# yahoo/bftkv

Measured on AMD Instinct MI355X. Metric: pgp_rsa2048_signature_verifies_per_sec, higher is better.
Workload: dtype u32; 1 GPU; 64-replica quorum, 10000 RSA-2048 signed writes per GPU (cfg2 of BASELINE.json), 534164 signature packets per GPU, 1.0% corrupt / 0.5% unknown issuer / 0.5% duplicate / 1.0% one-short; parallelism=shard-by-write x1, RCCL all-gather of verdict bitmaps on the verifier's stream, replicas=64, writes_per_gpu=10000, sigs_per_gpu=534164, batches_in_flight=3

## Files before the change

bftkv_amd/csrc/capi.hip:

```cpp
#include "../../include/bftkv_gpu.h"

#include <hip/hip_runtime.h>
#include <stdio.h>
#include <stdlib.h>
#include <string.h>

#include <limits.h>
#include <linux/futex.h>
#include <sched.h>
#include <sys/syscall.h>
#include <unistd.h>

#include <algorithm>
#include <array>
#include <atomic>
#include <memory>
#include <functional>
#include <map>
#include <set>
#include <chrono>
#include <condition_variable>
#include <mutex>
#include <shared_mutex>
#include <system_error>
// ... 163 lines not shown
  DevBuf txt_mid32, txt_mid64, txt_tail, txt_len;
  DevBuf forced_iss;
  DevBuf counts, base, total, item_flags, walk_scratch, cert_ent, sig_class, mid, mid64, hash_mask, recs, digests, r, xr, pk_list, pk_list3072, pk_list4096, r3072, r4096, pk_count, dsa_list, dsa_u, ids_tmp;
  DevBuf o_err, o_nver, o_verdict, o_fenced;
  DevBuf in_tbs, in_tbs_off, in_ss, in_ss_off;
  hipEvent_t seg_ev = nullptr;
  DevBuf in_prefix, in_prefix_off, in_shared, in_shared_off, in_seg;
  DevBuf st_tmp, item_tmp, bits_tmp, plan_cut;
  DevBuf chunk_arena, chunk_ctr;
  uint32_t multiexp_parts = 0;
  uint32_t ec_split = 0;
  uint32_t ec_window = 0;
  DevBuf ec_fb_tab[4];
  uint32_t ec_fb_w[4] = {};
  uint32_t multiexp_block = 0;
  uint32_t multiexp_lanes = 0;
  uint32_t rsav_lanes = 0;
  uint32_t dsa_inv_mode = 0;
  bool psign_caller_order = false;
  uint32_t n_cus = 256;
  uint32_t lagrange_x_bound = 0;
  bool early_exit = true;
  std::vector<DevBuf*> scratch_pool;
  std::unordered_map<std::string, std::vector<uint32_t>> modrow_cache;
  std::unordered_map<std::string, std::vector<uint32_t>> rsav_row_cache[2];
  std::map<std::string, std::array<DevBuf, 4>> modtab_cache;
  uint32_t* h_mail = nullptr;
  uint32_t* d_mail = nullptr;
  uint32_t last_total = 0, last_rsa = 0, last_items = 0;
  bool last_total_on_dev = false;
  hipEvent_t ev[10] = {};
  hipEvent_t ev_turn = nullptr;
  bool have_timing = false;
  void* rccl_comm = nullptr;
  int n_ranks = 1, rank = 0;

  bftkv_gpu_ctx* root = nullptr;
  std::shared_mutex kt_rw;
  std::atomic<int> kt_writers{0};
  std::atomic<int> n_forks{0};
  uint64_t quorum_gen = 0;
  uint64_t seen_keyring_gen = ~0ull, seen_quorum_gen = ~0ull;
  size_t n_dsa_slots = 0;
  int kt_read_depth = 0;
  DevBuf in_pack;
  uint8_t* h_out = nullptr; uint8_t* d_out = nullptr; size_t out_cap = 0;
  uint32_t out_seq = 0;
  std::vector<bftkv_gpu_ctx*> hb_workers;
  hipStream_t stream_c = nullptr;
  hipStream_t stream_c2 = nullptr;
  std::vector<hipEvent_t> hb_ev;
  uint8_t* hb_out = nullptr; size_t hb_out_cap = 0;
  uint32_t modexp_lds_pad = 0;
  uint32_t hb_pieces = 0;
  hipEvent_t hb_ev0 = nullptr;
  bool hb_tight = false;
  uint32_t hb_copy_mode = 0;
  void* hb_ring = nullptr;
  std::vector<float> hb_trace;
  uint32_t hb_last_pieces = 0;
  std::vector<uint32_t> hb_item0;
  void* small_pin = nullptr;
  uint32_t staged_spin_us = 50000;
};

void rccl_release(bftkv_gpu_ctx* c);
void release_small_pin(bftkv_gpu_ctx* c);
extern "C" int signature_verify_entities(bftkv_gpu_ctx* c, uint32_t n_items, const uint8_t* tbs, const uint64_t* tbs_off, const uint8_t* sig,
                                         const uint64_t* sig_off, const uint32_t* ent, uint8_t* err_out, const uint8_t* sig_class = nullptr,
                                         uint8_t* fenced_out = nullptr, const uint64_t* forced_issuer = nullptr);

namespace {

int fork_refresh(bftkv_gpu_ctx* c);

struct KtWrite {
  bftkv_gpu_ctx* c;
  explicit KtWrite(bftkv_gpu_ctx* c_) : c(c_) { c->kt_writers.fetch_add(1); c->kt_rw.lock(); }
  ~KtWrite() { c->kt_rw.unlock(); c->kt_writers.fetch_sub(1); }
};
struct KtRead {
  bftkv_gpu_ctx *c, *r;
  int rc = 0;
  explicit KtRead(bftkv_gpu_ctx* c_) : c(c_), r(c_->root) {
    if (!r || c->kt_read_depth++ > 0) return;
    while (r->kt_writers.load(std::memory_order_acquire) > 0) std::this_thread::yield();
    r->kt_rw.lock_shared();
    rc = fork_refresh(c);
  }
  ~KtRead() { if (r && --c->kt_read_depth == 0) r->kt_rw.unlock_shared(); }
};

struct Turnstile { std::mutex mu; hipEvent_t last = nullptr; const void* owner = nullptr; };
Turnstile g_turnstile[16];
constexpr uint64_t HB_PIPE_MIN_BYTES = 24ull << 20;
constexpr uint32_t HB_PIPE_MAX_PIECES = 8;
std::mutex g_hb_mu[16];
constexpr size_t HB_TR = 10;
struct HbRing {
  static constexpr size_t SLOT = 16u << 20;
  static constexpr int NSLOT = 6;
  static constexpr int THREADS = 4;
  uint8_t* base = nullptr;
  hipEvent_t ev[NSLOT] = {};
  bool used[NSLOT] = {};
  ~HbRing() { if (base) (void)hipHostFree(base); for (auto e : ev) if (e) (void)hipEventDestroy(e); }
// ... 276 lines not shown
  }
  uint32_t* const cnt_p = c->pk_count.as<uint32_t>();
  const uint32_t* const start0 = cnt_p + 12;
  PlanArgs pl{};
  if (total && plan_q) {
    pl.recs = c->recs.as<SigRec>(); pl.rec_base = c->base.as<uint32_t>(); pl.counts = c->counts.as<uint32_t>(); pl.n_items = n_items;
    pl.pk_list = c->pk_list.as<uint32_t>(); pl.dsa_list = c->dsa_list.as<uint32_t>(); pl.pk_list3072 = c->pk_list3072.as<uint32_t>();
    pl.pk_list4096 = c->pk_list4096.as<uint32_t>(); pl.pk_count = cnt_p; pl.plan_cut = c->plan_cut.as<uint32_t>(); pl.verdict = nullptr;
    int min_suff = 0;
    for (int i = 0; i < plan_q->n_qcs; ++i) if (plan_q->suff[i] > 0 && (min_suff == 0 || plan_q->suff[i] < min_suff)) min_suff = plan_q->suff[i];
    pl.margin = 1u + (uint32_t)min_suff / 64u;
    pl.mail = c->d_mail ? c->d_mail + 3 : nullptr;
    if (c->h_mail) __atomic_store_n(&c->h_mail[3], 0u, __ATOMIC_RELEASE);
    hipLaunchKernelGGL(k_plan<1>, dim3((n_items + PLAN_ITEMS - 1) / PLAN_ITEMS), dim3(PLAN_BLOCK), 0, s, pl, c->kt, *plan_q);
  }
  const bool dsa_side = total && c->have_dsa_keys;
  if (one_stream && dsa_side) HIPCHK(c, hipEventRecord(c->ev[1], s)); else HIPCHK(c, rec(1, s));
  const size_t n_slots = c->root ? c->n_dsa_slots : c->dsa_comb_slot.size();
  const uint32_t inv_batch_min = c->dsa_inv_mode == 1 || n_slots > (c->dsa_inv_mode == 2 ? (size_t)INV_MAX_SLOTS : 256) ? 0xFFFFFFFFu
                                 : c->dsa_inv_mode == 2 ? 0u : (uint32_t)std::max<size_t>(4096, 64 * n_slots);
  auto launch_dsa_inv = [&](hipStream_t st, const uint32_t* start) {
    if (inv_batch_min != 0xFFFFFFFFu)
      hipLaunchKernelGGL(k_dsa_inv_batched, dim3((total + INV_TILE - 1) / INV_TILE), dim3(INV_BLOCK), 0, st, d_ss, c->recs.as<SigRec>(),
                         c->dsa_list.as<uint32_t>(), c->pk_count.as<uint32_t>(), start, c->kt, c->dsa_u.as<uint32_t>(), inv_batch_min);
    if (inv_batch_min != 0u)
      hipLaunchKernelGGL(k_dsa_inv, dim3((total + 63) / 64), dim3(64), 0, st, d_ss, c->recs.as<SigRec>(), c->dsa_list.as<uint32_t>(),
                         c->pk_count.as<uint32_t>(), start, c->kt, c->dsa_u.as<uint32_t>(), inv_batch_min);
  };
  if (total && c->have_dsa_keys) {
    HIPCHK(c, hipStreamWaitEvent(c->stream_d, c->ev[1], 0));
    launch_dsa_inv(c->stream_d, start0);
    HIPCHK(c, hipEventRecord(c->ev[7], c->stream_d));
  }
  auto hash_stream_work = [&]() -> int {
    HIPCHK(c, join(sh, 1));
    if (total) {
      if (!d_mid_in) {
        hipLaunchKernelGGL(k_hash_mid_other, dim3((n_items + 63) / 64, N_HASHES - 1), dim3(64), 0, sh, d_tbs, d_tbs_off, n_items,
                           c->hash_mask.as<uint32_t>(), c->mid.as<uint32_t>(), c->mid64.as<uint64_t>());
        hipLaunchKernelGGL(k_hash_mid_text, dim3((n_items + 63) / 64, N_HASHES), dim3(64), 0, sh, d_tbs, d_tbs_off, n_items, c->hash_mask.as<uint32_t>(), txt);
      }
      hipLaunchKernelGGL(k_digest_sha256, dim3((total + 255) / 256), dim3(256), 0, sh, d_tbs, d_tbs_off, d_ss,
                         d_mid_in ? d_mid_in : c->mid.as<uint32_t>(), c->mid64.as<uint64_t>(), n_items, c->recs.as<SigRec>(), total,
                         c->digests.as<uint32_t>(), d_tbs_prefix, n_recs_dev);
    }
    HIPCHK(c, rec(6, sh));
    return 0;
  };
  if (!upload_tbs) { int hrc = hash_stream_work(); if (hrc) return hrc; }
  const dim3 qg((total + MODEXP_BLOCK / MONT_TPI - 1) / (MODEXP_BLOCK / MONT_TPI));
  const dim3 qg8((total + MODEXP_BLOCK / MONT_TPI_BIG - 1) / (MODEXP_BLOCK / MONT_TPI_BIG));
  static const bool wide8_off = getenv("BFTKV_NO_WIDE8") != nullptr;
  const bool wide8 = staged_cap != 0 && ss_len / 256 <= 8192 && !wide8_off;
  auto launch_modexp = [&](const uint32_t* start) {
    if (wide8)
      hipLaunchKernelGGL((k_rsa_modexp<10, MONT_TPI_BIG>), qg8, dim3(MODEXP_BLOCK), 0, s, d_ss, c->recs.as<SigRec>(), c->pk_list.as<uint32_t>(),
                         cnt_p, start, c->kt, c->r.as<uint32_t>(), c->xr.as<uint32_t>(), (uint64_t*)(cnt_p + 16));
    else {
#if BFTKV_RSA_FORM == 29
      hipLaunchKernelGGL((k_rsa_modexp<RSA29_L, MONT_TPI, RSA29_W>), qg, dim3(MODEXP_BLOCK), c->modexp_lds_pad, s, d_ss, c->recs.as<SigRec>(), c->pk_list.as<uint32_t>(),
                         cnt_p, start, c->kt, c->r.as<uint32_t>(), c->xr.as<uint32_t>(), (uint64_t*)(cnt_p + 16), (const uint32_t*)(cnt_p + 5));
      hipLaunchKernelGGL((k_rsa_modexp<MONT_L, MONT_TPI, MONT_W, true>), qg, dim3(MODEXP_BLOCK), c->modexp_lds_pad, s, d_ss, c->recs.as<SigRec>(), c->pk_list.as<uint32_t>(),
                         cnt_p, start, c->kt, c->r.as<uint32_t>(), c->xr.as<uint32_t>(), (uint64_t*)nullptr, (const uint32_t*)(cnt_p + 5));
#else
      hipLaunchKernelGGL((k_rsa_modexp<MONT_L, MONT_TPI>), qg, dim3(MODEXP_BLOCK), c->modexp_lds_pad, s, d_ss, c->recs.as<SigRec>(), c->pk_list.as<uint32_t>(),
                         cnt_p, start, c->kt, c->r.as<uint32_t>(), c->xr.as<uint32_t>(), (uint64_t*)(cnt_p + 16));
#endif
    }
    if (c->have_rsa3072)
      hipLaunchKernelGGL((k_rsa_modexp<MONT_L3072, MONT_TPI_BIG>), qg8, dim3(MODEXP_BLOCK), 0, s, d_ss, c->recs.as<SigRec>(), c->pk_list3072.as<uint32_t>(),
                         cnt_p + 2, start + 2, c->kt, c->r3072.as<uint32_t>(), c->xr.as<uint32_t>(), (uint64_t*)nullptr);
    if (c->have_rsa4096)
      hipLaunchKernelGGL((k_rsa_modexp<MONT_L4096, MONT_TPI_BIG>), qg8, dim3(MODEXP_BLOCK), 0, s, d_ss, c->recs.as<SigRec>(), c->pk_list4096.as<uint32_t>(),
                         cnt_p + 3, start + 3, c->kt, c->r4096.as<uint32_t>(), c->xr.as<uint32_t>(), (uint64_t*)nullptr);
  };
  static const bool turnstile_off = getenv("BFTKV_NO_TURNSTILE") != nullptr;
  const bool big = staged_cap ? (ev_input != nullptr && ss_len / 320 >= TURNSTILE_MIN_PACKETS) : total >= TURNSTILE_MIN_PACKETS;
  if (big && !turnstile_off) {
    Turnstile& g = g_turnstile[(unsigned)c->device & 15u];
    std::lock_guard<std::mutex> tl(g.mu);
    if (g.last && g.owner != c) HIPCHK(c, hipStreamWaitEvent(s, g.last, 0));
    HIPCHK(c, rec(9, s));
    launch_modexp(start0);
    if (!c->ev_turn) HIPCHK(c, hipEventCreateWithFlags(&c->ev_turn, hipEventDisableTiming));
    HIPCHK(c, hipEventRecord(c->ev_turn, s));
    g.last = c->ev_turn; g.owner = c;
  } else {
    HIPCHK(c, rec(9, s));
    if (total) launch_modexp(start0);
  }
  HIPCHK(c, rec(2, s));
  if (upload_tbs) {
    int hrc = (*upload_tbs)(sh);
    if (hrc) return hrc;
    if (!mid_prelaunched)
      hipLaunchKernelGGL(k_sha256_mid, dim3((n_items + 63) / 64), dim3(64), 0, sh, d_tbs, d_tbs_off, n_items, c->mid.as<uint32_t>());
    if ((hrc = hash_stream_work())) return hrc;
  }
  HIPCHK(c, join(s, 6));
  bool other_hashes = true;
  if (total && !d_mid_in && plan_q && big && c->h_mail) {
    const auto t_spin = std::chrono::steady_clock::now();
    for (uint32_t it = 0;; ++it) {
      const uint32_t v = __atomic_load_n(&c->h_mail[3], __ATOMIC_ACQUIRE);
      if (v) { other_hashes = (v & 1u) != 0; break; }
      if ((it & 255u) == 255u && std::chrono::steady_clock::now() - t_spin > std::chrono::microseconds(300) + std::chrono::nanoseconds((uint64_t)total / 2)) break;
      __builtin_ia32_pause();
    }
  }
  if (total && !d_mid_in && other_hashes)
    hipLaunchKernelGGL(k_digest_other, dim3(std::min<uint32_t>((total + 255) / 256, DIGEST_OTHER_MAX_BLOCKS)), dim3(256), 0, s,
                       d_tbs, d_tbs_off, d_ss, c->mid.as<uint32_t>(), c->mid64.as<uint64_t>(), n_items, c->recs.as<SigRec>(), total,
                       c->digests.as<uint32_t>(), c->pk_count.as<uint32_t>() + 4, txt, n_recs_dev);
  const dim3 cg(((uint64_t)total * CMP_LANES + 255) / 256);
  auto launch_compare = [&](const uint32_t* start) {
    hipLaunchKernelGGL(k_rsa_compare, cg, dim3(256), 0, s, c->recs.as<SigRec>(), c->pk_list.as<uint32_t>(),
                       cnt_p, start, c->kt, c->r.as<uint32_t>(), c->digests.as<uint32_t>());
    if (c->have_rsa3072)
      hipLaunchKernelGGL(k_rsa_compare, cg, dim3(256), 0, s, c->recs.as<SigRec>(), c->pk_list3072.as<uint32_t>(),
                         cnt_p + 2, start + 2, c->kt, c->r3072.as<uint32_t>(), c->digests.as<uint32_t>());
    if (c->have_rsa4096)
      hipLaunchKernelGGL(k_rsa_compare, cg, dim3(256), 0, s, c->recs.as<SigRec>(), c->pk_list4096.as<uint32_t>(),
                         cnt_p + 3, start + 3, c->kt, c->r4096.as<uint32_t>(), c->digests.as<uint32_t>());
  };
  auto launch_dsa = [&](const uint32_t* start) {
    hipLaunchKernelGGL(k_dsa_mul, dim3((total + 63) / 64), dim3(64), 0, s, c->recs.as<SigRec>(), c->dsa_list.as<uint32_t>(),
                       cnt_p, start, c->kt, c->digests.as<uint32_t>(), c->dsa_u.as<uint32_t>());
    const uint32_t* idx_s = nullptr; const uint32_t* idx_b = nullptr; const uint32_t* cnt_cls = nullptr;
    if (c->have_dsa3072 && c->have_dsa2048) {
      uint32_t* cc = cnt_p + (start == start0 ? 20 : 22);
      uint32_t* is = c->dsa_idx.as<uint32_t>() + (start == start0 ? 0 : 2 * (size_t)total);
      hipLaunchKernelGGL(k_dsa_split, dim3((total + 255) / 256), dim3(256), 0, s, c->recs.as<SigRec>(), c->dsa_list.as<uint32_t>(), cnt_p, start, c->kt,
                         is, is + total, cc);
      idx_s = is; idx_b = is + total; cnt_cls = cc;
    }
    if (c->have_dsa2048)
      hipLaunchKernelGGL((k_dsa_modexp<MONT_L, MONT_TPI>), dim3((total + QUADS_PER_BLOCK - 1) / QUADS_PER_BLOCK), dim3(RSA_BLOCK), 0, s,
                         c->recs.as<SigRec>(), c->dsa_list.as<uint32_t>(), cnt_p, start, c->kt, c->dsa_u.as<uint32_t>(), idx_s, cnt_cls);
    if (c->have_dsa3072)
      hipLaunchKernelGGL((k_dsa_modexp<MONT_L3072, MONT_TPI_BIG>), dim3((total + RSA_BLOCK / MONT_TPI_BIG - 1) / (RSA_BLOCK / MONT_TPI_BIG)), dim3(RSA_BLOCK), 0, s,
                         c->recs.as<SigRec>(), c->dsa_list.as<uint32_t>(), cnt_p, start, c->kt, c->dsa_u.as<uint32_t>(), idx_b, cnt_cls ? cnt_cls + 1 : nullptr);
  };
  if (total) launch_compare(start0);
  HIPCHK(c, rec(8, s));
  if (total && c->have_dsa_keys) {
    HIPCHK(c, hipStreamWaitEvent(s, c->ev[7], 0));
    launch_dsa(start0);
  }
  if (total && plan_q) {
    HIPCHK(c, c->o_nver.ensure(sizeof(uint32_t) * n_items));
    HIPCHK(c, c->o_verdict.ensure(n_items));
    hipLaunchKernelGGL(k_tally, dim3((n_items + 3) / 4), dim3(256), 0, s, c->recs.as<SigRec>(), c->base.as<uint32_t>(), c->counts.as<uint32_t>(),
                       n_items, c->kt, *plan_q, c->o_verdict.as<uint8_t>(), c->o_nver.as<uint32_t>(), (uint32_t*)nullptr);
    hipLaunchKernelGGL(k_plan_snapshot, dim3(1), dim3(64), 0, s, cnt_p);
    pl.verdict = c->o_verdict.as<uint8_t>();
    hipLaunchKernelGGL(k_plan<2>, dim3((n_items + PLAN_ITEMS - 1) / PLAN_ITEMS), dim3(PLAN_BLOCK), 0, s, pl, c->kt, *plan_q);
    const uint32_t* const start1 = cnt_p + 8;
    if (c->have_dsa_keys) launch_dsa_inv(s, start1);
    launch_modexp(start1);
    launch_compare(start1);
    if (c->have_dsa_keys) launch_dsa(start1);
  }
  if (total && c->have_ambiguous && !d_msg_slot)
    hipLaunchKernelGGL(k_candidates, dim3((total + 63) / 64), dim3(64), 0, s, d_tbs, d_tbs_off, d_ss, d_mid_in ? d_mid_in : c->mid.as<uint32_t>(),
                       c->mid64.as<uint64_t>(), n_items, c->recs.as<SigRec>(), total, n_recs_dev, d_tbs_prefix, c->kt, d_cert_ent, d_sig_class, txt,
                       c->hash_mask.as<uint32_t>());
  HIPCHK(c, rec(3, s));
  HIPCHK(c, hipGetLastError());
  return 0;
}

int make_key_entry(bftkv_gpu_ctx* c, const bftkv_gpu_pubkey& k, bool cert_only, KeyEntry* out) {
  KeyEntry& e = *out;
  e.key_id = k.key_id; e.entity_id = k.entity_id; e.algo = k.pk_algo; e.cert_only = cert_only;
  e.material.clear();
  e.material.push_back((char)k.pk_algo);
  e.material.push_back((char)k.usable_sign);
  auto app = [&](const uint8_t* p, uint32_t l) {
    uint32_t z = 0;
    while (z < l && p[z] == 0) ++z;
    if (l > z) e.material.append((const char*)p + z, l - z);
    e.material.push_back('|');
  };
  app(k.n, k.n_len); app(k.e, k.e_len); app(k.g, k.g_len); app(k.y, k.y_len);
  e.flags = 0;
  if (k.usable_sign) e.flags |= KEYF_USABLE_SIGN;
  if (k.pk_algo != PK_RSA_ENCRYPT_ONLY && k.pk_algo != PK_ELGAMAL) e.flags |= KEYF_CAN_SIGN;
  if (k.key_id == k.entity_id) e.flags |= KEYF_PRIMARY;
  if (cert_only) e.flags |= KEYF_CERT_ONLY;
  e.bits = (uint32_t)hostbn::bit_length(k.n, k.n_len);
  e.e = 0; e.n0 = 0; e.qbits = 0;
  e.r2w.clear(); e.nl29.clear(); e.r2_29.clear(); e.n0_29 = 0;
  e.nl.assign(MONT_NMAX, 0); e.r2.assign(MONT_NMAX, 0); e.qw.assign(8, 0); e.dtab.assign(2 * DSA_N_BIG, 0); e.qpow.clear(); e.qconst.clear();
  if (k.pk_algo == PK_RSA || k.pk_algo == PK_RSA_SIGN_ONLY) {
    if (hostbn::bit_length(k.e, k.e_len) > 32) return fail(c, BFTKV_E_UNSUPPORTED, "RSA public exponent wider than 32 bits");
    for (uint32_t j = 0; j < k.e_len; ++j) e.e = (e.e << 8) | k.e[j];
    const int nlimbs = e.bits <= 2048 ? MONT_N : (e.bits <= 3072 ? MONT_TPI_BIG * MONT_L3072 : MONT_TPI_BIG * MONT_L4096);
    if (e.bits > 4096) e.bits = 0xFFFFFFFFu;
    else if (!hostbn::mont_setup(k.n, k.n_len, nlimbs, e.nl.data(), e.r2.data(), &e.n0)) e.bits = 0xFFFFFFFFu;
    else if (e.bits <= 2048) {
      std::vector<uint32_t> nl80(80);
      uint32_t n0b = 0;
      e.r2w.assign(80, 0);
      (void)hostbn::mont_setup(k.n, k.n_len, 80, nl80.data(), e.r2w.data(), &n0b);
      e.nl29.assign(RSA29_N, 0); e.r2_29.assign(RSA29_N, 0);
      (void)hostbn::mont_setup(k.n, k.n_len, RSA29_N, e.nl29.data(), e.r2_29.data(), &e.n0_29, RSA29_W);
    }
  } else if (k.pk_algo == PK_DSA) {
    e.qbits = (uint32_t)hostbn::bit_length(k.e, k.e_len);
    const int NLp = e.bits <= 2048 ? (int)DSA_N_SMALL : (int)DSA_N_BIG;
    const uint32_t cap_bits = e.bits <= 2048 ? 2048u : 3072u;
    const int nwords = (28 * NLp + 31) / 32 + 1;
    std::vector<uint32_t> p(nwords), g(nwords), y(nwords), q(nwords);
// ... 329 lines not shown
    c->keyring_gen = r->keyring_gen;
    c->seen_keyring_gen = r->keyring_gen;
  }
  c->early_exit = r->early_exit;
  if (c->seen_quorum_gen != r->quorum_gen) {
    for (auto& q : c->quorums) { q.member.release(); q.ids.release(); }
    c->quorums.clear();
    c->quorums.resize(r->quorums.size());
    for (size_t i = 0; i < r->quorums.size(); ++i) {
      const QuorumHost& s = r->quorums[i];
      QuorumHost& d = c->quorums[i];
      d.live = s.live; d.n_qcs = s.n_qcs; d.nodes = s.nodes;
      for (int k = 0; k < MAX_QC; ++k) { d.f[k] = s.f[k]; d.mn[k] = s.mn[k]; d.thr[k] = s.thr[k]; d.suff[k] = s.suff[k]; }
      d.keyring_gen = ~0ull;
    }
    c->seen_quorum_gen = r->quorum_gen;
  }
  return 0;
}

int check_offsets(bftkv_gpu_ctx* c, const uint64_t* off, uint32_t n, const char* what) {
  if (off[0] != 0) return fail(c, BFTKV_E_INVALID, what);
  for (uint32_t i = 0; i < n; ++i) if (off[i + 1] < off[i]) return fail(c, BFTKV_E_INVALID, what);
  return 0;
}

int check_quorum(bftkv_gpu_ctx* c, int quorum) {
  if (quorum < 0 || (size_t)quorum >= c->quorums.size() || !c->quorums[quorum].live) return fail(c, BFTKV_E_INVALID, "bad quorum handle");
  return 0;
}

}

extern "C" {

int bftkv_gpu_init(int device_ordinal, bftkv_gpu_ctx** out) {
  if (!out) return BFTKV_E_INVALID;
  int n = 0;
  if (hipGetDeviceCount(&n) != hipSuccess || n <= 0) return BFTKV_E_DEVICE;
  if (device_ordinal < 0 || device_ordinal >= n) return BFTKV_E_INVALID;
  if (hipSetDevice(device_ordinal) != hipSuccess) return BFTKV_E_DEVICE;
  bftkv_gpu_ctx* c = new bftkv_gpu_ctx();
  c->device = device_ordinal;
  if (hipHostMalloc((void**)&c->h_mail, 64, hipHostMallocMapped) == hipSuccess) {
    if (hipHostGetDevicePointer((void**)&c->d_mail, c->h_mail, 0) != hipSuccess) { (void)hipHostFree(c->h_mail); c->h_mail = nullptr; c->d_mail = nullptr; }
    else memset(c->h_mail, 0, 64);
  } else c->h_mail = nullptr;
  if (hipStreamCreateWithFlags(&c->stream, hipStreamNonBlocking) != hipSuccess ||
      hipStreamCreateWithFlags(&c->stream_h, hipStreamNonBlocking) != hipSuccess ||
      hipStreamCreateWithFlags(&c->stream_d, hipStreamNonBlocking) != hipSuccess) { delete c; return BFTKV_E_DEVICE; }
  { std::lock_guard<std::mutex> lk(g_live_mu); g_live.push_back(c); }
  if (const char* e = getenv("BFTKV_STAGED_SPIN_US")) c->staged_spin_us = (uint32_t)atoi(e);
  if (const char* e = getenv("BFTKV_MODEXP_LDS_PAD")) c->modexp_lds_pad = (uint32_t)atoi(e);
  if (const char* e = getenv("BFTKV_MULTIEXP_PARTS")) c->multiexp_parts = (uint32_t)atoi(e);
  if (const char* e = getenv("BFTKV_EC_SPLIT")) c->ec_split = (uint32_t)atoi(e);
  if (const char* e = getenv("BFTKV_EC_WINDOW")) c->ec_window = (uint32_t)atoi(e);
  if (const char* e = getenv("BFTKV_MULTIEXP_LANES")) c->multiexp_lanes = (uint32_t)atoi(e);
  if (const char* e = getenv("BFTKV_RSAV_LANES")) c->rsav_lanes = (uint32_t)atoi(e);
  if (const char* e = getenv("BFTKV_MULTIEXP_BLOCK")) c->multiexp_block = (uint32_t)atoi(e);
  if (const char* e = getenv("BFTKV_DSA_INV")) c->dsa_inv_mode = !strcmp(e, "batched") ? 2u : !strcmp(e, "single") ? 1u : 0u;
  if (const char* e = getenv("BFTKV_PSIGN_ORDER")) c->psign_caller_order = !strcmp(e, "caller");
  { int cus = 0; if (hipDeviceGetAttribute(&cus, hipDeviceAttributeMultiprocessorCount, device_ordinal) == hipSuccess && cus > 0) c->n_cus = (uint32_t)cus; }
  *out = c;
  return BFTKV_OK;
}

int bftkv_gpu_ctx_fork(bftkv_gpu_ctx* root, bftkv_gpu_ctx** out) {
  if (!root || !out) return BFTKV_E_INVALID;
  if (root->root) return fail(root, BFTKV_E_INVALID, "fork of a fork");
  bftkv_gpu_ctx* c = nullptr;
  int rc = bftkv_gpu_init(root->device, &c);
  if (rc) return rc;
  c->root = root;
  c->early_exit = root->early_exit;
  c->dsa_inv_mode = root->dsa_inv_mode;
  root->n_forks.fetch_add(1);
  *out = c;
  return 0;
}

void bftkv_gpu_destroy(bftkv_gpu_ctx* c) {
  if (!c) return;
  for (bftkv_gpu_ctx* w : c->hb_workers) bftkv_gpu_destroy(w);
  c->hb_workers.clear();
  if (!c->root && c->n_forks.load() > 0) {
    fprintf(stderr, "bftkv_gpu_destroy: context still has %d forked context(s); not destroyed\n", c->n_forks.load());
    return;
  }
  {
    std::lock_guard<std::mutex> lk(g_live_mu);
    for (size_t i = 0; i < g_live.size(); ++i) if (g_live[i] == c) { g_live.erase(g_live.begin() + i); break; }
  }
  (void)hipSetDevice(c->device);
  (void)hipStreamSynchronize(c->stream);
  (void)hipStreamSynchronize(c->stream_h);
  (void)hipStreamSynchronize(c->stream_d);
  for (DevBuf* b : {&c->k_id, &c->k_entity, &c->k_algo, &c->k_flags, &c->k_bits, &c->k_e, &c->k_n, &c->k_r2, &c->k_n0, &c->k_q, &c->k_qbits, &c->k_dsatab, &c->k_dsaslot, &c->dsa_comb, &c->k_sorted_id, &c->k_sorted_slot, &c->k_r2w, &c->k_n29, &c->k_r2_29, &c->k_n0_29,
                    &c->chunk_arena, &c->chunk_ctr, &c->counts, &c->base, &c->total, &c->item_flags, &c->walk_scratch, &c->cert_ent, &c->sig_class, &c->mid, &c->mid64, &c->hash_mask, &c->recs, &c->digests, &c->r, &c->xr,
                    &c->pk_list, &c->pk_list3072, &c->pk_list4096, &c->r3072, &c->r4096, &c->pk_count, &c->dsa_list, &c->dsa_u, &c->dsa_idx, &c->ids_tmp, &c->o_err, &c->o_nver, &c->o_verdict, &c->o_fenced, &c->in_tbs, &c->in_tbs_off,
                    &c->in_ss, &c->in_ss_off, &c->in_prefix, &c->in_prefix_off, &c->in_shared, &c->in_shared_off, &c->in_seg, &c->st_tmp, &c->item_tmp, &c->bits_tmp, &c->plan_cut, &c->txt_mid32, &c->txt_mid64, &c->txt_tail, &c->txt_len})
    b->release();
  for (auto& q : c->quorums) { q.member.release(); q.ids.release(); }
  keysets_release_all(c);
  c->in_pack.release();
  c->forced_iss.release();
  release_small_pin(c);
  if (c->h_out) (void)hipHostFree(c->h_out);
  if (c->root) c->root->n_forks.fetch_sub(1);
  for (DevBuf* b : c->scratch_pool) { b->release(); delete b; }
  for (auto& kv : c->modtab_cache) for (DevBuf& b : kv.second) b.release();
  for (DevBuf& b : c->ec_fb_tab) b.release();
  if (c->h_mail) (void)hipHostFree(c->h_mail);
  if (c->hb_out) (void)hipHostFree(c->hb_out);
  if (c->hb_ring) { if (c->stream_c) (void)hipStreamSynchronize(c->stream_c); delete (HbRing*)c->hb_ring; }
  for (hipEvent_t e : c->hb_ev) (void)hipEventDestroy(e);
  if (c->hb_ev0) (void)hipEventDestroy(c->hb_ev0);
  if (c->seg_ev) (void)hipEventDestroy(c->seg_ev);
  if (c->stream_c) { (void)hipStreamSynchronize(c->stream_c); (void)hipStreamDestroy(c->stream_c); }
  if (c->stream_c2) { (void)hipStreamSynchronize(c->stream_c2); (void)hipStreamDestroy(c->stream_c2); }
  rccl_release(c);
  for (auto& e : c->ev) if (e) (void)hipEventDestroy(e);
  if (c->ev_turn) {
    Turnstile& g = g_turnstile[(unsigned)c->device & 15u];
    std::lock_guard<std::mutex> tl(g.mu);
    if (g.owner == c) { g.last = nullptr; g.owner = nullptr; }
    (void)hipEventDestroy(c->ev_turn);
  }
  (void)hipStreamDestroy(c->stream);
// ... 943 lines not shown
```

bftkv_amd/csrc/kernels.hip:

```cpp
#include <hip/hip_runtime.h>
#include <stdint.h>

#include "device_types.h"
#include "mont28.h"
#include "value_load.h"
#include "u256.h"
#include "hashes.h"

namespace bftkv {

struct ParsedPacket {
  uint64_t next;
  bool event;
  SigRec rec;
};

__host__ __device__ __forceinline__ bool known_tag(uint32_t tag) {
  return tag < 32 && ((0x00066BFEu >> tag) & 1u);
}

struct SubpacketState {
  bool have_ctime = false, have_issuer = false, have_embedded = false;
  bool too_deep = false;
  uint64_t issuer = 0;
// ... 1239 lines not shown
      kind = (bitpos >= 0) ? OP_SQR : OP_MUL1;
    }
    canonicalize<L, TPI, W>(y, qlane);
    if (e_u == 0) {
#pragma unroll
      for (int k = 0; k < L; ++k) y[k] = (qlane == 0 && k == 0) ? 1u : 0u;
    }
    uint32_t head = 0;
    if constexpr (W == MONT_W) {
#pragma unroll
      for (int k = 0; k < L; ++k) {
        const uint32_t gi = (uint32_t)qlane * L + k;
        if (gi >= (uint32_t)EM_LOW_LIMBS) head |= y[k] ^ em_head_limb(gi, kbytes);
      }
    } else {
#pragma unroll
      for (int k = 0; k < L; ++k) {
        const int32_t lo = ((int32_t)qlane * L + k) * W, cut = 8 * EM_LOW_BYTES;
        if (lo + W > cut) {
          const uint32_t d = y[k] ^ em_head_limb<W>((uint32_t)qlane * L + k, kbytes);
          head |= (lo < cut) ? d >> (cut - lo) : d;
        }
      }
    }
    head = grp_or<TPI>(head);
    if (W == MONT_W && head != 0 && qlane == 0) y[0] = EM_HEAD_BAD;
#pragma unroll
    for (int k = 0; k < L; ++k) a_lds[k] = y[k];
    __builtin_amdgcn_fence(__ATOMIC_ACQ_REL, "wavefront");
    if (live && active && qlane < 4) {
      uint32_t* out = r_low + (uint64_t)pi * EM_LOW_LIMBS + qlane * (EM_LOW_LIMBS / 4);
      if constexpr (W == MONT_W) {
        const uint32_t* src = a_rd + qlane * (EM_LOW_LIMBS / 4);
#pragma unroll
        for (int k = 0; k < EM_LOW_LIMBS / 4; ++k) out[k] = src[k];
      } else {
#pragma unroll
        for (int k = 0; k < EM_LOW_LIMBS / 4; ++k) {
          const uint32_t bit = (uint32_t)MONT_W * ((uint32_t)qlane * (EM_LOW_LIMBS / 4) + k), i = bit / W, sh = bit % W;
          const uint32_t v = ((a_rd[i] >> sh) | (a_rd[i + 1] << (W - sh))) & MONT_MASK;
          out[k] = (head != 0 && qlane == 0 && k == 0) ? EM_HEAD_BAD : v;
        }
      }
    }
    __builtin_amdgcn_fence(__ATOMIC_ACQ_REL, "wavefront");
    todo &= ~__builtin_amdgcn_ballot_w64(live);
  }
  if (stamp && *pk_start_ptr == 0) { clk[0] = __builtin_readcyclecounter() - t0; clk[1] = __builtin_amdgcn_s_memrealtime() - r0; }
}

constexpr int CMP_LANES = 4;
constexpr int CMP_L = EM_LOW_LIMBS / CMP_LANES;
static_assert(CMP_L * CMP_LANES == EM_LOW_LIMBS, "the low limbs divide over the quad");
__global__ void __launch_bounds__(256) k_rsa_compare(SigRec* __restrict__ recs, const uint32_t* __restrict__ pk_list,
                                                     const uint32_t* __restrict__ pk_count_ptr, const uint32_t* __restrict__ pk_start_ptr,
                                                     KeyTableDev kt,
                                                     const uint32_t* __restrict__ r_low, const uint32_t* __restrict__ digests) {
  constexpr int GROUPS = 256 / CMP_LANES;
  const uint32_t count = *pk_count_ptr, start = *pk_start_ptr;
  const uint32_t q0 = start + blockIdx.x * GROUPS;
  if (q0 >= count) return;
  const uint32_t gq = q0 + threadIdx.x / CMP_LANES;
  const int qlane = threadIdx.x % CMP_LANES;
  const bool active = gq < count;
  const uint32_t pi = active ? gq : (count - 1);
  const uint32_t ri = pk_list[pi];
  const SigRec rec = recs[ri];
  const bool pending = rec.status == ST_PENDING_RSA;
  const uint32_t key = (uint32_t)rec.key_slot;
  const uint32_t kbytes = (kt.mod_bits[key] + 7) >> 3;
  const HashInfo hi = hash_info(rec.hash_id);
  const uint32_t hlen = hi.dlen, plen = hi.plen, tl = hlen + plen;
  constexpr int EM_TAIL_W = 24;
  __shared__ uint32_t tail_sh[GROUPS * EM_TAIL_W];
  uint32_t* tail = tail_sh + (threadIdx.x / CMP_LANES) * EM_TAIL_W;
  const uint32_t* dgw = digests + (uint64_t)ri * 16;
  const uint32_t hw = hlen >> 2;
#pragma unroll
  for (int t = 0; t < EM_TAIL_W / CMP_LANES; ++t) {
    const uint32_t w = (uint32_t)qlane * (EM_TAIL_W / CMP_LANES) + t;
    uint32_t v = 0;
    if (w < hw) v = __builtin_bswap32(dgw[hw - 1 - w]);
    else {
#pragma unroll
      for (uint32_t bq = 0; bq < 4; ++bq) {
        const uint32_t i = 4 * w + bq;
        if (i >= hlen && i < tl) v |= digestinfo_byte(rec.hash_id, plen - 1 - (i - hlen)) << (8 * bq);
      }
    }
    tail[w] = v;
  }
  __builtin_amdgcn_fence(__ATOMIC_ACQ_REL, "wavefront");
  auto em_word = [&](uint32_t w) -> uint32_t {
    if (4 * w + 3 <= tl) return tail[w];
    if (4 * w > tl && 4 * w + 3 + 2 < kbytes) return 0xFFFFFFFFu;
    uint32_t v = 0;
#pragma unroll
    for (uint32_t bq = 0; bq < 4; ++bq) {
      const uint32_t i = 4 * w + bq;
      uint32_t byte;
      if (i <= tl) byte = (tail[i >> 2] >> (8 * (i & 3))) & 0xFFu;
      else if (i + 2 < kbytes) byte = 0xFF;
      else byte = (i + 2 == kbytes) ? 1u : 0u;
      v |= byte << (8 * bq);
    }
    return v;
  };
  constexpr int NW = (CMP_L * MONT_W + 31) / 32 + 1;
  const uint32_t bit0 = (uint32_t)qlane * CMP_L * MONT_W, w0 = bit0 >> 5, s0 = bit0 & 31u;
  uint32_t Wd[NW + 1], Wn[NW];
#pragma unroll
  for (int i = 0; i <= NW; ++i) Wd[i] = em_word(w0 + i);
#pragma unroll
  for (int i = 0; i < NW; ++i) Wn[i] = __builtin_amdgcn_alignbit(Wd[i + 1], Wd[i], s0);
  __shared__ uint32_t r_sh[GROUPS * EM_LOW_LIMBS];
  {
    const uint32_t n_valid = min((uint32_t)GROUPS, count - q0) * EM_LOW_LIMBS;
    const uint32_t* src = r_low + (uint64_t)q0 * EM_LOW_LIMBS;
    for (uint32_t t = threadIdx.x; t < GROUPS * EM_LOW_LIMBS; t += 256) r_sh[t] = t < n_valid ? src[t] : 0u;
    __syncthreads();
  }
  const uint32_t* rp = r_sh + (threadIdx.x / CMP_LANES) * EM_LOW_LIMBS + qlane * CMP_L;
  uint32_t diff = 0;
#pragma unroll
  for (int k = 0; k < CMP_L; ++k) {
    const int bit = MONT_W * k, wi = bit >> 5, sh = bit & 31;
    const uint32_t em = (sh == 0 ? Wn[wi] : __builtin_amdgcn_alignbit(Wn[wi + 1], Wn[wi], sh)) & MONT_MASK;
    diff |= em ^ rp[k];
  }
  diff = quad_or(diff);
  if (active && pending && qlane == 0) recs[ri].status = (diff == 0) ? ST_OK : ST_BAD_SIG;
}

constexpr int DSA_U_WORDS = 24;
__device__ __forceinline__ const uint32_t* dsa_slot_base(const KeyTableDev& kt, uint32_t key) {
  return kt.dsa_comb + (uint64_t)kt.dsa_slot[key] * dsa_slot_stride(kt.dsa_wbits, kt.dsa_entry_limbs);
}
__device__ __forceinline__ const uint32_t* dsa_qconst(const KeyTableDev& kt, uint32_t key) {
  return dsa_slot_base(kt, key) + dsa_comb_limbs_per_key(kt.dsa_wbits, kt.dsa_entry_limbs) + dsa_qpow_words(kt.dsa_entry_limbs);
}
__global__ void __launch_bounds__(64) k_dsa_inv(const uint8_t* __restrict__ sig_blob, const SigRec* __restrict__ recs,
                                                const uint32_t* __restrict__ dsa_list, const uint32_t* __restrict__ pk_count,
                                                const uint32_t* __restrict__ pk_start,
                                                KeyTableDev kt, uint32_t* __restrict__ dsa_u , uint32_t batch_min) {
  if (pk_count[1] - pk_start[1] >= batch_min) return;
  const uint32_t di = pk_start[1] + blockIdx.x * blockDim.x + threadIdx.x;
  if (di >= pk_count[1]) return;
  const uint32_t ri = dsa_list[di];
  const uint32_t key = (uint32_t)recs[ri].key_slot;
  const uint64_t body_off = recs[ri].body_off;
  const uint32_t off0 = recs[ri].mpi_off[0], off1 = recs[ri].mpi_off[1], bits0 = recs[ri].mpi_bits[0], bits1 = recs[ri].mpi_bits[1];
  U256 q, r, s_, w;
  for (int i = 0; i < 8; ++i) q.w[i] = kt.q_words[(uint64_t)key * 8 + i];
  const uint32_t qbits = kt.q_bits[key];
  const uint8_t* body = sig_blob + body_off;
  bool ok = u256_from_be(body + off0, (bits0 + 7u) >> 3, r);
  ok = u256_from_be(body + off1, (bits1 + 7u) >> 3, s_) && ok;
  ok = ok && !u256_is_zero(r) && u256_cmp(r, q) < 0 && !u256_is_zero(s_) && u256_cmp(s_, q) < 0;
  ok = ok && (qbits & 7u) == 0;
  ok = ok && u256_modinv_odd(s_, q, w);
  U256 u2 = u256_zero();
  if (ok) {
    const uint32_t* qc = dsa_qconst(kt, key);
    U256 r2;
    for (int i = 0; i < 8; ++i) r2.w[i] = qc[i];
    u2 = u256_mulmod_mont(w, r, q, qc[8], r2);
  } else w = u256_zero();
  uint32_t* o = dsa_u + (uint64_t)di * DSA_U_WORDS;
  for (int i = 0; i < 8; ++i) { o[i] = w.w[i]; o[8 + i] = u2.w[i]; o[16 + i] = r.w[i]; }
}

constexpr int INV_BLOCK = 256, INV_PER_THREAD = 16, INV_TILE = INV_BLOCK * INV_PER_THREAD, INV_MAX_SLOTS = 4096;
__global__ void __launch_bounds__(INV_BLOCK) k_dsa_inv_batched(const uint8_t* __restrict__ sig_blob, const SigRec* __restrict__ recs,
                                                               const uint32_t* __restrict__ dsa_list, const uint32_t* __restrict__ pk_count,
                                                               const uint32_t* __restrict__ pk_start,
                                                               KeyTableDev kt, uint32_t* __restrict__ dsa_u , uint32_t batch_min) {
  if (pk_count[1] - pk_start[1] < batch_min) return;
  __shared__ uint32_t bins[INV_MAX_SLOTS];
  __shared__ uint32_t tsum[INV_BLOCK];
  __shared__ uint16_t order[INV_TILE], slot_of[INV_TILE];
  const uint32_t count = pk_count[1], start = pk_start[1];
  const uint32_t tile0 = start + blockIdx.x * INV_TILE;
  if (tile0 >= count) return;
  const uint32_t n = min((uint32_t)INV_TILE, count - tile0);
// ... 496 lines not shown
    const uint64_t okm = __builtin_amdgcn_ballot_w64(ok);
    const uint64_t below = (lane == 0) ? 0ull : (~0ull >> (64 - lane));
    bool reached = false;
#pragma unroll
    for (int c = 0; c < MAX_QC; ++c) {
      if (c < q.n_qcs) {
        const bool mem = ok && q.member[(uint64_t)c * q.n_entities + ent];
        const uint64_t mm = __builtin_amdgcn_ballot_w64(mem);
        const uint32_t run = cq[c] + (uint32_t)__builtin_popcountll(mm & below) + (mem ? 1u : 0u);
        if (ok && q.suff[c] > 0 && run >= (uint32_t)q.suff[c]) reached = true;
        cq[c] += (uint32_t)__builtin_popcountll(mm);
      }
    }
    const uint64_t rm = __builtin_amdgcn_ballot_w64(reached);
    if (rm != 0 && first_suff == 0xFFFFFFFFu) {
      const uint32_t fl = (uint32_t)__builtin_ctzll(rm);
      first_suff = total_ok + (uint32_t)__builtin_popcountll(okm & ((fl == 63) ? ~0ull : ((1ull << (fl + 1)) - 1)));
    }
    total_ok += (uint32_t)__builtin_popcountll(okm);
  }
  if (lane == 0) {
    bool is_quorum = q.n_qcs > 0, is_thr = q.n_qcs > 0, is_suff = false, reject = true;
    for (int c = 0; c < q.n_qcs; ++c) {
      if (q.f[c] > 0 && (int32_t)cq[c] < q.min[c]) is_quorum = false;
      if (q.threshold[c] > 0 && (int32_t)cq[c] < q.threshold[c]) is_thr = false;
      if (q.suff[c] > 0 && (int32_t)cq[c] >= q.suff[c]) is_suff = true;
      if (q.f[c] == 0 || (int32_t)cq[c] <= q.f[c]) reject = false;
    }
    verdict[wave] = (is_quorum ? V_IS_QUORUM : 0) | (is_thr ? V_IS_THRESHOLD : 0) | (is_suff ? V_IS_SUFFICIENT : 0) |
                    (reject ? V_REJECT : 0);
    n_verified[wave] = is_suff ? first_suff : total_ok;
    if (clique_counts)
      for (int c = 0; c < MAX_QC; ++c) clique_counts[(uint64_t)wave * MAX_QC + c] = cq[c];
  }
}

struct PlanArgs {
  SigRec* recs; const uint32_t* rec_base; const uint32_t* counts; uint32_t n_items;
  uint32_t *pk_list, *dsa_list, *pk_list3072, *pk_list4096;
  uint32_t* pk_count;
  uint32_t* plan_cut;
  const uint8_t* verdict;
  uint32_t margin;
  uint32_t* mail;
};

constexpr int PLAN_BLOCK = 1024, PLAN_ITEMS = PLAN_BLOCK / 64;
template <int PHASE>
__global__ void __launch_bounds__(PLAN_BLOCK) k_plan(PlanArgs a, KeyTableDev kt, QuorumDev q) {
  __shared__ uint32_t cnt_sh[PLAN_ITEMS][4];
  const uint32_t wib = threadIdx.x >> 6, lane = threadIdx.x & 63;
  const uint32_t item = blockIdx.x * PLAN_ITEMS + wib;
  if (PHASE == 1 && a.mail && blockIdx.x == 0 && threadIdx.x == 0)
    __hip_atomic_store(a.mail, 0x80000000u | (a.pk_count[4] ? 1u : 0u), __ATOMIC_RELEASE, __HIP_MEMORY_SCOPE_SYSTEM);
  const bool have = item < a.n_items;
  const uint32_t base = have ? a.rec_base[item] : 0, cnt = have ? a.counts[item] : 0;
  uint32_t* const lists[4] = {a.pk_list, a.dsa_list, a.pk_list3072, a.pk_list4096};
  const uint64_t below = (lane == 0) ? 0ull : (~0ull >> (64 - lane));
  uint32_t from = 0, covered = cnt;
  if (PHASE == 1) {
    uint32_t cq[MAX_QC];
#pragma unroll
    for (int c = 0; c < MAX_QC; ++c) cq[c] = 0;
    bool done = false;
    for (uint32_t off = 0; off < cnt && !done; off += 64) {
      const uint32_t i = off + lane;
      uint32_t kind = 0, ent = 0;
      if (i < cnt) {
        kind = a.recs[base + i].q_kind1;
        if (kind) ent = kt.entity[a.recs[base + i].key_slot];
      }
      bool reached = false;
#pragma unroll
      for (int c = 0; c < MAX_QC; ++c) {
        if (c < q.n_qcs) {
          const bool mem = kind != 0 && q.member[(uint64_t)c * q.n_entities + ent];
          const uint64_t mm = __builtin_amdgcn_ballot_w64(mem);
          const uint32_t run = cq[c] + (uint32_t)__builtin_popcountll(mm & below) + (mem ? 1u : 0u);
          if (mem && q.suff[c] > 0 && run >= (uint32_t)q.suff[c] + a.margin) reached = true;
          cq[c] += (uint32_t)__builtin_popcountll(mm);
        }
      }
      const uint64_t rm = __builtin_amdgcn_ballot_w64(reached);
      if (rm) { done = true; covered = off + (uint32_t)__builtin_ctzll(rm) + 1; }
    }
  } else {
    from = have ? a.plan_cut[item] : 0;
    if (!have || (a.verdict[item] & V_IS_SUFFICIENT)) from = covered;
  }
  auto wants = [&](uint32_t i, uint32_t& kind) -> bool {
    kind = 0;
    if (i >= covered) return false;
    if (PHASE == 1) { kind = a.recs[base + i].q_kind1; return kind != 0; }
    const SigRec r = a.recs[base + i];
    kind = r.q_kind1;
    return kind != 0 && !r.queued && r.status == ST_PENDING_RSA;
  };
  uint32_t n_k[4] = {0, 0, 0, 0};
  for (uint32_t off = from; off < covered; off += 64) {
    uint32_t kind;
    const bool w = wants(off + lane, kind);
#pragma unroll
    for (int k = 0; k < 4; ++k) n_k[k] += (uint32_t)__builtin_popcountll(__builtin_amdgcn_ballot_w64(w && kind == (uint32_t)k + 1));
  }
  if (lane == 0) {
#pragma unroll
    for (int k = 0; k < 4; ++k) cnt_sh[wib][k] = n_k[k];
// ... 100 lines not shown
```

Before: 163.7 million verifies/s.

## Defer wide RSA modexp pass behind host mail flag and bound phase-2 compare grid

The second (wide-value fallback) RSA-29 modexp launch is moved out of the first launch batch. It now runs only when the plan kernel's mail word reports that wide values exist (pk_count[5] nonzero). In phase 2, the compare kernel gets a grid-stride variant capped at a few blocks per CU, so it does not launch many mostly-empty blocks over the dynamic count. This saves launching a kernel that often has no work and trims idle blocks, but it makes the wide pass wait on the host spin-read of the mail flag. If the flag times out, wide_values stays true and the pass still runs.

```diff
diff --git a/bftkv_amd/csrc/capi.hip b/bftkv_amd/csrc/capi.hip
--- a/bftkv_amd/csrc/capi.hip
+++ b/bftkv_amd/csrc/capi.hip
@@ -239,6 +239,7 @@
   std::vector<hipEvent_t> hb_ev;
   uint8_t* hb_out = nullptr; size_t hb_out_cap = 0;
   uint32_t modexp_lds_pad = 0;
+  uint32_t phase2_blocks = 0;
   uint32_t hb_pieces = 0;
   hipEvent_t hb_ev0 = nullptr;
   bool hb_tight = false;
@@ -621,6 +622,22 @@
   const dim3 qg8((total + MODEXP_BLOCK / MONT_TPI_BIG - 1) / (MODEXP_BLOCK / MONT_TPI_BIG));
   static const bool wide8_off = getenv("BFTKV_NO_WIDE8") != nullptr;
   const bool wide8 = staged_cap != 0 && ss_len / 256 <= 8192 && !wide8_off;
+#ifdef BFTKV_FULL_GRIDS
+  constexpr bool bounded_grids = false;
+#else
+  constexpr bool bounded_grids = true;
+#endif
+  const uint32_t grid_bound = c->phase2_blocks ? c->phase2_blocks : 3u * c->n_cus;
+  auto bounded = [&](const dim3& g) { return dim3(std::min<uint32_t>(g.x, grid_bound)); };
+  auto launch_wide = [&](const uint32_t* start) {
+#if BFTKV_RSA_FORM == 29
+    if (!wide8)
+      hipLaunchKernelGGL((k_rsa_modexp<MONT_L, MONT_TPI, MONT_W, true>), qg, dim3(MODEXP_BLOCK), c->modexp_lds_pad, s, d_ss, c->recs.as<SigRec>(), c->pk_list.as<uint32_t>(),
+                         cnt_p, start, c->kt, c->r.as<uint32_t>(), c->xr.as<uint32_t>(), (uint64_t*)nullptr, (const uint32_t*)(cnt_p + 5));
+#else
+    (void)start;
+#endif
+  };
   auto launch_modexp = [&](const uint32_t* start) {
     if (wide8)
       hipLaunchKernelGGL((k_rsa_modexp<10, MONT_TPI_BIG>), qg8, dim3(MODEXP_BLOCK), 0, s, d_ss, c->recs.as<SigRec>(), c->pk_list.as<uint32_t>(),
@@ -629,8 +646,7 @@
 #if BFTKV_RSA_FORM == 29
       hipLaunchKernelGGL((k_rsa_modexp<RSA29_L, MONT_TPI, RSA29_W>), qg, dim3(MODEXP_BLOCK), c->modexp_lds_pad, s, d_ss, c->recs.as<SigRec>(), c->pk_list.as<uint32_t>(),
                          cnt_p, start, c->kt, c->r.as<uint32_t>(), c->xr.as<uint32_t>(), (uint64_t*)(cnt_p + 16), (const uint32_t*)(cnt_p + 5));
-      hipLaunchKernelGGL((k_rsa_modexp<MONT_L, MONT_TPI, MONT_W, true>), qg, dim3(MODEXP_BLOCK), c->modexp_lds_pad, s, d_ss, c->recs.as<SigRec>(), c->pk_list.as<uint32_t>(),
-                         cnt_p, start, c->kt, c->r.as<uint32_t>(), c->xr.as<uint32_t>(), (uint64_t*)nullptr, (const uint32_t*)(cnt_p + 5));
+      if (!bounded_grids) launch_wide(start);
 #else
       hipLaunchKernelGGL((k_rsa_modexp<MONT_L, MONT_TPI>), qg, dim3(MODEXP_BLOCK), c->modexp_lds_pad, s, d_ss, c->recs.as<SigRec>(), c->pk_list.as<uint32_t>(),
                          cnt_p, start, c->kt, c->r.as<uint32_t>(), c->xr.as<uint32_t>(), (uint64_t*)(cnt_p + 16));
@@ -667,30 +683,32 @@
     if ((hrc = hash_stream_work())) return hrc;
   }
   HIPCHK(c, join(s, 6));
-  bool other_hashes = true;
+  bool other_hashes = true, wide_values = true;
   if (total && !d_mid_in && plan_q && big && c->h_mail) {
     const auto t_spin = std::chrono::steady_clock::now();
     for (uint32_t it = 0;; ++it) {
       const uint32_t v = __atomic_load_n(&c->h_mail[3], __ATOMIC_ACQUIRE);
-      if (v) { other_hashes = (v & 1u) != 0; break; }
+      if (v) { other_hashes = (v & 1u) != 0; wide_values = (v & 2u) != 0; break; }
       if ((it & 255u) == 255u && std::chrono::steady_clock::now() - t_spin > std::chrono::microseconds(300) + std::chrono::nanoseconds((uint64_t)total / 2)) break;
       __builtin_ia32_pause();
     }
   }
+  if (total && bounded_grids && wide_values) launch_wide(start0);
   if (total && !d_mid_in && other_hashes)
     hipLaunchKernelGGL(k_digest_other, dim3(std::min<uint32_t>((total + 255) / 256, DIGEST_OTHER_MAX_BLOCKS)), dim3(256), 0, s,
                        d_tbs, d_tbs_off, d_ss, c->mid.as<uint32_t>(), c->mid64.as<uint64_t>(), n_items, c->recs.as<SigRec>(), total,
                        c->digests.as<uint32_t>(), c->pk_count.as<uint32_t>() + 4, txt, n_recs_dev);
   const dim3 cg(((uint64_t)total * CMP_LANES + 255) / 256);
-  auto launch_compare = [&](const uint32_t* start) {
-    hipLaunchKernelGGL(k_rsa_compare, cg, dim3(256), 0, s, c->recs.as<SigRec>(), c->pk_list.as<uint32_t>(),
-                       cnt_p, start, c->kt, c->r.as<uint32_t>(), c->digests.as<uint32_t>());
-    if (c->have_rsa3072)
-      hipLaunchKernelGGL(k_rsa_compare, cg, dim3(256), 0, s, c->recs.as<SigRec>(), c->pk_list3072.as<uint32_t>(),
-                         cnt_p + 2, start + 2, c->kt, c->r3072.as<uint32_t>(), c->digests.as<uint32_t>());
-    if (c->have_rsa4096)
-      hipLaunchKernelGGL(k_rsa_compare, cg, dim3(256), 0, s, c->recs.as<SigRec>(), c->pk_list4096.as<uint32_t>(),
-                         cnt_p + 3, start + 3, c->kt, c->r4096.as<uint32_t>(), c->digests.as<uint32_t>());
+  auto compare_list = [&](bool phase2, const uint32_t* list, const uint32_t* cnt, const uint32_t* start, const uint32_t* r_low) {
+    if (bounded_grids && phase2)
+      hipLaunchKernelGGL(k_rsa_compare<true>, bounded(cg), dim3(256), 0, s, c->recs.as<SigRec>(), list, cnt, start, c->kt, r_low, c->digests.as<uint32_t>());
+    else
+      hipLaunchKernelGGL(k_rsa_compare<false>, cg, dim3(256), 0, s, c->recs.as<SigRec>(), list, cnt, start, c->kt, r_low, c->digests.as<uint32_t>());
+  };
+  auto launch_compare = [&](const uint32_t* start, bool phase2) {
+    compare_list(phase2, c->pk_list.as<uint32_t>(), cnt_p, start, c->r.as<uint32_t>());
+    if (c->have_rsa3072) compare_list(phase2, c->pk_list3072.as<uint32_t>(), cnt_p + 2, start + 2, c->r3072.as<uint32_t>());
+    if (c->have_rsa4096) compare_list(phase2, c->pk_list4096.as<uint32_t>(), cnt_p + 3, start + 3, c->r4096.as<uint32_t>());
   };
   auto launch_dsa = [&](const uint32_t* start) {
     hipLaunchKernelGGL(k_dsa_mul, dim3((total + 63) / 64), dim3(64), 0, s, c->recs.as<SigRec>(), c->dsa_list.as<uint32_t>(),
@@ -710,7 +728,7 @@
       hipLaunchKernelGGL((k_dsa_modexp<MONT_L3072, MONT_TPI_BIG>), dim3((total + RSA_BLOCK / MONT_TPI_BIG - 1) / (RSA_BLOCK / MONT_TPI_BIG)), dim3(RSA_BLOCK), 0, s,
                          c->recs.as<SigRec>(), c->dsa_list.as<uint32_t>(), cnt_p, start, c->kt, c->dsa_u.as<uint32_t>(), idx_b, cnt_cls ? cnt_cls + 1 : nullptr);
   };
-  if (total) launch_compare(start0);
+  if (total) launch_compare(start0, false);
   HIPCHK(c, rec(8, s));
   if (total && c->have_dsa_keys) {
     HIPCHK(c, hipStreamWaitEvent(s, c->ev[7], 0));
@@ -727,7 +745,8 @@
     const uint32_t* const start1 = cnt_p + 8;
     if (c->have_dsa_keys) launch_dsa_inv(s, start1);
     launch_modexp(start1);
-    launch_compare(start1);
+    if (bounded_grids && wide_values) launch_wide(start1);
+    launch_compare(start1, true);
     if (c->have_dsa_keys) launch_dsa(start1);
   }
   if (total && c->have_ambiguous && !d_msg_slot)
@@ -1163,6 +1182,7 @@
   { std::lock_guard<std::mutex> lk(g_live_mu); g_live.push_back(c); }
   if (const char* e = getenv("BFTKV_STAGED_SPIN_US")) c->staged_spin_us = (uint32_t)atoi(e);
   if (const char* e = getenv("BFTKV_MODEXP_LDS_PAD")) c->modexp_lds_pad = (uint32_t)atoi(e);
+  if (const char* e = getenv("BFTKV_PHASE2_BLOCKS")) c->phase2_blocks = (uint32_t)std::max(0, atoi(e));
   if (const char* e = getenv("BFTKV_MULTIEXP_PARTS")) c->multiexp_parts = (uint32_t)atoi(e);
   if (const char* e = getenv("BFTKV_EC_SPLIT")) c->ec_split = (uint32_t)atoi(e);
   if (const char* e = getenv("BFTKV_EC_WINDOW")) c->ec_window = (uint32_t)atoi(e);
@@ -1185,6 +1205,7 @@
   c->root = root;
   c->early_exit = root->early_exit;
   c->dsa_inv_mode = root->dsa_inv_mode;
+  c->phase2_blocks = root->phase2_blocks;
   root->n_forks.fetch_add(1);
   *out = c;
   return 0;
diff --git a/bftkv_amd/csrc/kernels.hip b/bftkv_amd/csrc/kernels.hip
--- a/bftkv_amd/csrc/kernels.hip
+++ b/bftkv_amd/csrc/kernels.hip
@@ -1315,84 +1315,89 @@
 constexpr int CMP_LANES = 4;
 constexpr int CMP_L = EM_LOW_LIMBS / CMP_LANES;
 static_assert(CMP_L * CMP_LANES == EM_LOW_LIMBS, "the low limbs divide over the quad");
+template <bool STRIDED = false>
 __global__ void __launch_bounds__(256) k_rsa_compare(SigRec* __restrict__ recs, const uint32_t* __restrict__ pk_list,
                                                      const uint32_t* __restrict__ pk_count_ptr, const uint32_t* __restrict__ pk_start_ptr,
                                                      KeyTableDev kt,
                                                      const uint32_t* __restrict__ r_low, const uint32_t* __restrict__ digests) {
   constexpr int GROUPS = 256 / CMP_LANES;
   const uint32_t count = *pk_count_ptr, start = *pk_start_ptr;
-  const uint32_t q0 = start + blockIdx.x * GROUPS;
-  if (q0 >= count) return;
-  const uint32_t gq = q0 + threadIdx.x / CMP_LANES;
-  const int qlane = threadIdx.x % CMP_LANES;
-  const bool active = gq < count;
-  const uint32_t pi = active ? gq : (count - 1);
-  const uint32_t ri = pk_list[pi];
-  const SigRec rec = recs[ri];
-  const bool pending = rec.status == ST_PENDING_RSA;
-  const uint32_t key = (uint32_t)rec.key_slot;
-  const uint32_t kbytes = (kt.mod_bits[key] + 7) >> 3;
-  const HashInfo hi = hash_info(rec.hash_id);
-  const uint32_t hlen = hi.dlen, plen = hi.plen, tl = hlen + plen;
-  constexpr int EM_TAIL_W = 24;
-  __shared__ uint32_t tail_sh[GROUPS * EM_TAIL_W];
-  uint32_t* tail = tail_sh + (threadIdx.x / CMP_LANES) * EM_TAIL_W;
-  const uint32_t* dgw = digests + (uint64_t)ri * 16;
-  const uint32_t hw = hlen >> 2;
-#pragma unroll
-  for (int t = 0; t < EM_TAIL_W / CMP_LANES; ++t) {
-    const uint32_t w = (uint32_t)qlane * (EM_TAIL_W / CMP_LANES) + t;
-    uint32_t v = 0;
-    if (w < hw) v = __builtin_bswap32(dgw[hw - 1 - w]);
-    else {
+  for (uint32_t blk = blockIdx.x;; blk += gridDim.x) {
+    const uint32_t q0 = start + blk * GROUPS;
+    if (q0 >= count) return;
+    const uint32_t gq = q0 + threadIdx.x / CMP_LANES;
+    const int qlane = threadIdx.x % CMP_LANES;
+    const bool active = gq < count;
+    const uint32_t pi = active ? gq : (count - 1);
+    const uint32_t ri = pk_list[pi];
+    const SigRec rec = recs[ri];
+    const bool pending = rec.status == ST_PENDING_RSA;
+    const uint32_t key = (uint32_t)rec.key_slot;
+    const uint32_t kbytes = (kt.mod_bits[key] + 7) >> 3;
+    const HashInfo hi = hash_info(rec.hash_id);
+    const uint32_t hlen = hi.dlen, plen = hi.plen, tl = hlen + plen;
+    constexpr int EM_TAIL_W = 24;
+    __shared__ uint32_t tail_sh[GROUPS * EM_TAIL_W];
+    uint32_t* tail = tail_sh + (threadIdx.x / CMP_LANES) * EM_TAIL_W;
+    const uint32_t* dgw = digests + (uint64_t)ri * 16;
+    const uint32_t hw = hlen >> 2;
+#pragma unroll
+    for (int t = 0; t < EM_TAIL_W / CMP_LANES; ++t) {
+      const uint32_t w = (uint32_t)qlane * (EM_TAIL_W / CMP_LANES) + t;
+      uint32_t v = 0;
+      if (w < hw) v = __builtin_bswap32(dgw[hw - 1 - w]);
+      else {
+#pragma unroll
+        for (uint32_t bq = 0; bq < 4; ++bq) {
+          const uint32_t i = 4 * w + bq;
+          if (i >= hlen && i < tl) v |= digestinfo_byte(rec.hash_id, plen - 1 - (i - hlen)) << (8 * bq);
+        }
+      }
+      tail[w] = v;
+    }
+    __builtin_amdgcn_fence(__ATOMIC_ACQ_REL, "wavefront");
+    auto em_word = [&](uint32_t w) -> uint32_t {
+      if (4 * w + 3 <= tl) return tail[w];
+      if (4 * w > tl && 4 * w + 3 + 2 < kbytes) return 0xFFFFFFFFu;
+      uint32_t v = 0;
 #pragma unroll
       for (uint32_t bq = 0; bq < 4; ++bq) {
         const uint32_t i = 4 * w + bq;
-        if (i >= hlen && i < tl) v |= digestinfo_byte(rec.hash_id, plen - 1 - (i - hlen)) << (8 * bq);
-      }
-    }
-    tail[w] = v;
-  }
-  __builtin_amdgcn_fence(__ATOMIC_ACQ_REL, "wavefront");
-  auto em_word = [&](uint32_t w) -> uint32_t {
-    if (4 * w + 3 <= tl) return tail[w];
-    if (4 * w > tl && 4 * w + 3 + 2 < kbytes) return 0xFFFFFFFFu;
-    uint32_t v = 0;
-#pragma unroll
-    for (uint32_t bq = 0; bq < 4; ++bq) {
-      const uint32_t i = 4 * w + bq;
-      uint32_t byte;
-      if (i <= tl) byte = (tail[i >> 2] >> (8 * (i & 3))) & 0xFFu;
-      else if (i + 2 < kbytes) byte = 0xFF;
-      else byte = (i + 2 == kbytes) ? 1u : 0u;
-      v |= byte << (8 * bq);
-    }
-    return v;
-  };
-  constexpr int NW = (CMP_L * MONT_W + 31) / 32 + 1;
-  const uint32_t bit0 = (uint32_t)qlane * CMP_L * MONT_W, w0 = bit0 >> 5, s0 = bit0 & 31u;
-  uint32_t Wd[NW + 1], Wn[NW];
-#pragma unroll
-  for (int i = 0; i <= NW; ++i) Wd[i] = em_word(w0 + i);
-#pragma unroll
-  for (int i = 0; i < NW; ++i) Wn[i] = __builtin_amdgcn_alignbit(Wd[i + 1], Wd[i], s0);
-  __shared__ uint32_t r_sh[GROUPS * EM_LOW_LIMBS];
-  {
-    const uint32_t n_valid = min((uint32_t)GROUPS, count - q0) * EM_LOW_LIMBS;
-    const uint32_t* src = r_low + (uint64_t)q0 * EM_LOW_LIMBS;
-    for (uint32_t t = threadIdx.x; t < GROUPS * EM_LOW_LIMBS; t += 256) r_sh[t] = t < n_valid ? src[t] : 0u;
+        uint32_t byte;
+        if (i <= tl) byte = (tail[i >> 2] >> (8 * (i & 3))) & 0xFFu;
+        else if (i + 2 < kbytes) byte = 0xFF;
+        else byte = (i + 2 == kbytes) ? 1u : 0u;
+        v |= byte << (8 * bq);
+      }
+      return v;
+    };
+    constexpr int NW = (CMP_L * MONT_W + 31) / 32 + 1;
+    const uint32_t bit0 = (uint32_t)qlane * CMP_L * MONT_W, w0 = bit0 >> 5, s0 = bit0 & 31u;
+    uint32_t Wd[NW + 1], Wn[NW];
+#pragma unroll
+    for (int i = 0; i <= NW; ++i) Wd[i] = em_word(w0 + i);
+#pragma unroll
+    for (int i = 0; i < NW; ++i) Wn[i] = __builtin_amdgcn_alignbit(Wd[i + 1], Wd[i], s0);
+    __shared__ uint32_t r_sh[GROUPS * EM_LOW_LIMBS];
+    {
+      const uint32_t n_valid = min((uint32_t)GROUPS, count - q0) * EM_LOW_LIMBS;
+      const uint32_t* src = r_low + (uint64_t)q0 * EM_LOW_LIMBS;
+      for (uint32_t t = threadIdx.x; t < GROUPS * EM_LOW_LIMBS; t += 256) r_sh[t] = t < n_valid ? src[t] : 0u;
+      __syncthreads();
+    }
+    const uint32_t* rp = r_sh + (threadIdx.x / CMP_LANES) * EM_LOW_LIMBS + qlane * CMP_L;
+    uint32_t diff = 0;
+#pragma unroll
+    for (int k = 0; k < CMP_L; ++k) {
+      const int bit = MONT_W * k, wi = bit >> 5, sh = bit & 31;
+      const uint32_t em = (sh == 0 ? Wn[wi] : __builtin_amdgcn_alignbit(Wn[wi + 1], Wn[wi], sh)) & MONT_MASK;
+      diff |= em ^ rp[k];
+    }
+    diff = quad_or(diff);
+    if (active && pending && qlane == 0) recs[ri].status = (diff == 0) ? ST_OK : ST_BAD_SIG;
+    if constexpr (!STRIDED) return;
     __syncthreads();
   }
-  const uint32_t* rp = r_sh + (threadIdx.x / CMP_LANES) * EM_LOW_LIMBS + qlane * CMP_L;
-  uint32_t diff = 0;
-#pragma unroll
-  for (int k = 0; k < CMP_L; ++k) {
-    const int bit = MONT_W * k, wi = bit >> 5, sh = bit & 31;
-    const uint32_t em = (sh == 0 ? Wn[wi] : __builtin_amdgcn_alignbit(Wn[wi + 1], Wn[wi], sh)) & MONT_MASK;
-    diff |= em ^ rp[k];
-  }
-  diff = quad_or(diff);
-  if (active && pending && qlane == 0) recs[ri].status = (diff == 0) ? ST_OK : ST_BAD_SIG;
 }
 
 constexpr int DSA_U_WORDS = 24;
@@ -1995,7 +2000,7 @@
   const uint32_t wib = threadIdx.x >> 6, lane = threadIdx.x & 63;
   const uint32_t item = blockIdx.x * PLAN_ITEMS + wib;
   if (PHASE == 1 && a.mail && blockIdx.x == 0 && threadIdx.x == 0)
-    __hip_atomic_store(a.mail, 0x80000000u | (a.pk_count[4] ? 1u : 0u), __ATOMIC_RELEASE, __HIP_MEMORY_SCOPE_SYSTEM);
+    __hip_atomic_store(a.mail, 0x80000000u | (a.pk_count[4] ? 1u : 0u) | (a.pk_count[5] ? 2u : 0u), __ATOMIC_RELEASE, __HIP_MEMORY_SCOPE_SYSTEM);
   const bool have = item < a.n_items;
   const uint32_t base = have ? a.rec_base[item] : 0, cnt = have ? a.counts[item] : 0;
   uint32_t* const lists[4] = {a.pk_list, a.dsa_list, a.pk_list3072, a.pk_list4096};
```

After: 164.1 million verifies/s, median of 2. Within noise of the previous version (+0.2%).
